# jhollowed/PyTEMDiags

Hardware: AMD Instinct MI355X
Metric: grid-points/sec through full TEM pipeline (ncol*nlev*nt) (higher is better)
Workload: dtype f64; 1 GPU; ne120 (777602 cols) x 72 lev x 30 snapshots per GPU, L=50, 1-degree zonal grid (M=180), ten GM16 Table-A1 outputs; ncol=777602, nlev=72, nt=30, sweeps=latitude-class, single sweep, mirror_paired_sweeps=True

## Files before the change

include/temx.h:

```cpp
#ifndef TEMX_H
#define TEMX_H

#include <stdint.h>

#ifdef __cplusplus
extern "C" {
#endif

typedef struct temx_plan temx_plan;

enum { TEMX_F64 = 0, TEMX_F32 = 1 };

enum {
  TEMX_OK = 0,
  TEMX_EINVAL = -1,
  TEMX_EHIP = -2,
  TEMX_ENOMEM = -3,
  TEMX_ERANK = -4,
  TEMX_ESTATE = -5,
  TEMX_EUNSUPPORTED = -6,
  TEMX_EINTERNAL = -7
};

enum {
  TEMX_DEFER_FINALIZE = 1,
  TEMX_NO_SYMMETRY = 2,
  TEMX_NO_CLASSES = 4,
  TEMX_NO_QR = 8,
  TEMX_LAT_TOL_F32 = 16
};

enum {
  TEMX_OPT_FORM = 1,
  TEMX_OPT_OS_MAP = 2,
  TEMX_OPT_OP_MAP = 3,
  TEMX_OPT_OS_SUBSAMPLE = 4,
  TEMX_OPT_TRACER_ONE_PASS = 5,
  TEMX_OPT_SINGLE_SWEEP_MIN_GROUPS = 6,
  TEMX_OPT_OS_CONTRACT = 7,
  TEMX_OPT_MISSING = 8,
  TEMX_OPT_MIN_COVERAGE = 9,
  TEMX_OPT_MISSING_WEIGHT = 10,
  TEMX_OPT_LAT_BINS = 12,
  TEMX_OPT_BIN_DEGREE = 13,
  TEMX_OPT_OS_SYNC = 11
};
enum {
  TEMX_FORM_AUTO = -1,
  TEMX_FORM_TWO_PASS = 0,
  TEMX_FORM_CLASS_SUMS = 1,
  TEMX_FORM_SINGLE_SWEEP = 2,
  TEMX_FORM_NO_SINGLE_SWEEP = 3,
  TEMX_FORM_MASKED = 4,
  TEMX_FORM_BINNED = 5
};

enum {
  TEMX_MAT_Y0 = 0,
  TEMX_MAT_Y0P = 1,
  TEMX_MAT_GRAM = 2,
  TEMX_MAT_GINV = 3,
  TEMX_MAT_Y0INV = 4,
  TEMX_MAT_GRAM2 = 5,
  TEMX_MAT_GX = 6,
  TEMX_MAT_GSUB = 7,
  TEMX_MAT_COVERAGE = 8
};

enum {
  TEMX_R_VTEM = 0, TEMX_R_OMEGATEM, TEMX_R_WTEM, TEMX_R_PSITEM, TEMX_R_EPFY, TEMX_R_EPFZ,
  TEMX_R_EPDIV, TEMX_R_UTENDEPFD, TEMX_R_UTENDVTEM, TEMX_R_UTENDWTEM, TEMX_NRESULTS
};

enum {
  TEMX_Z_UB = 0, TEMX_Z_VB, TEMX_Z_THETAB, TEMX_Z_WAPB, TEMX_Z_UPVPB, TEMX_Z_UPWAPPB,
  TEMX_Z_VPTPB, TEMX_Z_DUB_DP, TEMX_Z_DTHETAB_DP, TEMX_Z_UBCOSLAT, TEMX_Z_DUBCOSLAT_DLAT,
  TEMX_Z_PSI, TEMX_Z_PSICOSLAT, TEMX_Z_DPSICOSLAT_DLAT, TEMX_Z_DPSI_DP, TEMX_Z_INT_VBDP,
  TEMX_NZONAL
};

enum {
  TEMX_E_UP = 0, TEMX_E_VP, TEMX_E_THETAP, TEMX_E_WAPP, TEMX_E_UPVP, TEMX_E_UPWAPP, TEMX_E_VPTP,
  TEMX_NEDDY
};

int temx_version(void);
const char* temx_last_error(void);
int temx_device_count(void);

int temx_plan_create(temx_plan** out, int device, int64_t ncol, int L, int M,
                     const double* lat_deg_host, const double* lat_out_deg_host, int flags);

int temx_plan_finalize(temx_plan* plan, const double* G_host );

int temx_plan_refine(temx_plan* plan, const double* G2_host );

int temx_plan_set_weights(temx_plan* plan, const double* weights_host );

// ... 106 lines not shown
```

pytemdiags_amd/_lib.py:

```python
from __future__ import annotations

import ctypes as C
import os

_HERE = os.path.dirname(os.path.abspath(__file__))
LIB_PATH = os.environ.get("TEMX_LIB") or os.path.join(_HERE, "libtemx.so")

ABI_VERSION = 402
F64, F32 = 0, 1
DEFER_FINALIZE = 1
NO_SYMMETRY = 2
NO_CLASSES = 4
NO_QR = 8
LAT_TOL_F32 = 16
MAT_Y0, MAT_Y0P, MAT_GRAM, MAT_GINV, MAT_Y0INV, MAT_GRAM2, MAT_GX, MAT_GSUB = 0, 1, 2, 3, 4, 5, 6, 7
MAT_COVERAGE = 8
OPT_FORM, OPT_OS_MAP, OPT_OP_MAP, OPT_OS_SUBSAMPLE, OPT_TRACER_ONE_PASS, OPT_SINGLE_SWEEP_MIN_GROUPS, OPT_OS_CONTRACT = 1, 2, 3, 4, 5, 6, 7
OPT_MISSING, OPT_MIN_COVERAGE, OPT_MISSING_WEIGHT = 8, 9, 10
OPT_OS_SYNC = 11
OPT_LAT_BINS, OPT_BIN_DEGREE = 12, 13
LAT_BINS_ALLOWED = (128, 256, 512, 1024, 2048)
LAT_BINS_DEFAULT = 512
MISSING_MODES = {"raise": 0, "mask": 1}
FORM_AUTO, FORM_TWO_PASS, FORM_CLASS_SUMS, FORM_SINGLE_SWEEP, FORM_NO_SINGLE_SWEEP = -1, 0, 1, 2, 3
FORM_MASKED = 4
FORM_BINNED = 5
FORM_NAMES = {FORM_TWO_PASS: "two-pass", FORM_CLASS_SUMS: "class-sums", FORM_SINGLE_SWEEP: "single-sweep",
              FORM_MASKED: "masked", FORM_BINNED: "binned"}
FORMS = {"auto": FORM_AUTO, "two-pass": FORM_TWO_PASS, "class-sums": FORM_CLASS_SUMS,
         "single-sweep": FORM_SINGLE_SWEEP, "no-single-sweep": FORM_NO_SINGLE_SWEEP}

RESULT_NAMES = ("vtem", "omegatem", "wtem", "psitem", "epfy", "epfz", "epdiv",
                "utendepfd", "utendvtem", "utendwtem")
ZONAL_NAMES = ("ub", "vb", "thetab", "wapb", "upvpb", "upwappb", "vptpb", "dub_dp", "dthetab_dp",
               "ubcoslat", "dubcoslat_dlat", "psi", "psicoslat", "dpsicoslat_dlat", "dpsi_dp",
               "int_vbdp")
EDDY_NAMES = ("up", "vp", "thetap", "wapp", "upvp", "upwapp", "vptp")
TRACER_RESULT_NAMES = ("etfy", "etfz", "etdiv", "qtendetfd", "qtendvtem", "qtendwtem")
TRACER_ZONAL_NAMES = ("qb", "qpvpb", "qpwappb", "dqb_dp", "qbcoslat", "dqbcoslat_dlat")
TRACER_EDDY_NAMES = ("qp", "qpvp", "qpwapp")

ERRORS = {0: "TEMX_OK", -1: "TEMX_EINVAL", -2: "TEMX_EHIP", -3: "TEMX_ENOMEM", -4: "TEMX_ERANK",
          -5: "TEMX_ESTATE", -6: "TEMX_EUNSUPPORTED", -7: "TEMX_EINTERNAL"}

_vp, _i, _i64, _dp, _u64 = C.c_void_p, C.c_int, C.c_int64, C.POINTER(C.c_double), C.c_uint64
SIGNATURES = [
    ("temx_version", _i, []),
    ("temx_last_error", C.c_char_p, []),
    ("temx_device_count", _i, []),
    ("temx_plan_create", _i, [C.POINTER(_vp), _i, _i64, _i, _i, _dp, _dp, _i]),
    ("temx_plan_finalize", _i, [_vp, _dp]),
    ("temx_plan_refine", _i, [_vp, _dp]),
    ("temx_plan_set_weights", _i, [_vp, _dp]),
    ("temx_plan_destroy", None, [_vp]),
    ("temx_plan_is_paired", _i, [_vp]),
    ("temx_plan_sweep_mode", _i, [_vp]),
    ("temx_plan_one_pass", _i, [_vp]),
    ("temx_plan_single_sweep", _i, [_vp]),
    ("temx_get_matrix", _i, [_vp, _i, _vp, _vp]),
    ("temx_plan_configure", _i, [_vp, _i, _i]),
    ("temx_plan_option", _i, [_vp, _i]),
    ("temx_plan_set_os_matrices", _i, [_vp, _dp, _dp]),
    ("temx_project", _i, [_vp, _vp, _i, _i64, _vp, _vp]),
    ("temx_zonal_mean", _i, [_vp, _vp, _i, _i64, _vp, _i, _vp]),
    ("temx_zonal_mean_from_sums", _i, [_vp, _vp, _i64, _vp, _i, _vp]),
    ("temx_plan_set_tem", _i, [_vp, _i, _i64, _dp, C.c_double]),
    ("temx_tem_stage1", _i, [_vp, _vp, _vp, _vp, _vp, _i, _vp, _vp]),
    ("temx_tem_stage2", _i, [_vp, _vp, _vp, _vp, _vp, _i, _vp, _vp, _vp]),
    ("temx_tem_stage2_from_sums", _i, [_vp, _vp, _vp, _vp]),
    ("temx_tem_stage3", _i, [_vp, _vp, _vp, _vp, _vp]),
    ("temx_tem_run", _i, [_vp, _vp, _vp, _vp, _vp, _i, _vp, _vp, _vp]),
# ... 95 lines not shown
```

pytemdiags_amd/csrc/kernels_op2.hpp:

```cpp
#pragma once
#include "kernels_op.hpp"

namespace temx {

template <int NA, int NB>
struct OpwSlot {
  double sd[2][NA][64];
  double y[NB * 16];
};

template <int TBS, int NA>
__device__ __forceinline__ void opw_round(const OpwSlot<NA, 2 * TBS>* slots, int par, int t0, int nbw,
                                          uint32_t yoff, int lane, double (&acc)[NA][(TBS + 1) / 2]) {
  asm volatile("s_waitcnt lgkmcnt(0)\n\ts_barrier" ::: "memory");
#pragma unroll
  for (int j = 0; j < 4; ++j) {
    double b[NA];
#pragma unroll
    for (int f = 0; f < NA; ++f) b[f] = slots[j].sd[par][f][lane];
#pragma unroll
    for (int tl = 0; tl < (TBS + 1) / 2; ++tl)
      if (tl < nbw) {
        const double ya = slots[j].y[(t0 + tl) * 16 + yoff];
#pragma unroll
// ... 907 lines not shown
    }
  };

  if (b0 < b1) {
    load_ys(grp);
    rn = crow[(int64_t)b0 * 4 + wave];
    static_for<PD - 1>([&](auto kc) __attribute__((always_inline)) {
      constexpr int k = decltype(kc)::value;
      const int4 r0 = rn;
      rn = crow[(int64_t)(b0 + k + 1) * 4 + wave];
      issue(kc, r0);
    });
    constexpr int UNR = PD % 4 == 0 ? PD : PD % 2 == 0 ? 2 * PD : 4 * PD;
    for (int b = b0; b < b1; b += UNR)
      static_for<UNR>([&](auto kc) __attribute__((always_inline)) {
        constexpr int k = decltype(kc)::value;
        if (k == 0 || b + k < b1) step(kc, b + k);
      });
    asm volatile("s_waitcnt vmcnt(0)" ::: "memory");
  }
  if constexpr (SYNC != 0) {
    if (hpend) {
      if (left > 0) {
        const int first = (b1 - b0) & (NCH - 1);
        static_for<NCH>([&](auto cc) __attribute__((always_inline)) {
          if (((decltype(cc)::value - first) & (NCH - 1)) < left) pending_chunk(cc);
        });
      }
      handoff_wait(&hctr[0], handoff_look(&hctr[0]), 4u * hgen, 1);
      tile_role(ypend);
    }
    if (hfail != 0 && lane == 0) atomicOr(hstat, hfail);
  }
  if (left > 0) {
    const int first = (b1 - b0) & (NCH - 1);
    static_for<NCH>([&](auto cc) __attribute__((always_inline)) {
      if (((decltype(cc)::value - first) & (NCH - 1)) < left) pending_chunk(cc);
    });
  }
  if (dvalid) {
#pragma unroll
    for (int f = 0; f < NFX; ++f)
#pragma unroll
      for (int t = 0; t < NBX; ++t) {
        const int l = symx_harm<TBX>(t, g);
        if (l < (pp != nullptr ? KX : K4)) px[(((int64_t)split * NFX + f) * KX + l) * D + d] = ax[f][t];
      }
#pragma unroll
    for (int k = 0; k < NP; ++k)
#pragma unroll
      for (int t = 0; t < 2 * TBS; ++t) {
        const int l = sym_harm<TBS>(t, g);
        if (pp != nullptr && l < K) pp[(((int64_t)split * NP + k) * K + l) * D + d] = k < NPR ? apr[k < NPR ? k : 0][t] : apl[((k < NPR ? 0 : k - NPR) * 2 * TBS + t) * 64];
      }
  }
}

#ifndef TEMX_OS2_STAGGER
#define TEMX_OS2_STAGGER 0
#endif
#ifndef TEMX_OS2_ACC32
#define TEMX_OS2_ACC32 1
#endif
template <typename T, int TBS, int TBX, int NBR, int PD, int KIND = 0>
__global__ void __launch_bounds__(512, 1)
sweep_os2_kernel(FieldPtrs<4> fp, int64_t D, int K, int KX, const double* __restrict__ ycx,
                 const int4* __restrict__ crowN, const int4* __restrict__ crowS,
                 const int* __restrict__ gfirstN, const int* __restrict__ gfirstS, const int2* __restrict__ csplit,
                 const double* __restrict__ colscale, const double* __restrict__ rho, int K4,
                 double* __restrict__ px, double* __restrict__ pp, int nsplit, int ndt) {
  using KD = OsKind<KIND>;
  constexpr int NF = KD::NF, NFX = KD::NFX, NP = KD::NP;
  constexpr int NBX = 2 * TBX;
  constexpr int YE = NBX * 16;
  constexpr int MB = CLS_MB;
  constexpr int NCH = 2;
  constexpr int NV = NF + NP;
  constexpr int NPR = KD::NPR, NPL = NP - NPR;
  static_assert(NBR <= TBS && TBS <= TBX, "reference degree <= L <= 2L");
  static_assert(YE <= 512, "one Y element per thread");
  static_assert((PD - 1) * MB * NF + (MB - 1) * NF + 1 <= 63, "the ring is counted in vmcnt (6 bits)");
  extern __shared__ double lds[];
  int split, dq;
  if (!wg_work((ndt + 3) / 4, nsplit, split, dq)) return;
  const int tid = threadIdx.x;
  const int wave = uniform_wave(), lane = tid & 63;
  const int c = lane & 15, g = lane >> 4;
  const int side = wave >> 2;
  const int64_t colr = (int64_t)dq * 64 + lane < D ? (int64_t)dq * 64 + lane : D - 1;
  const uint32_t colb32 = (uint32_t)colr * (uint32_t)sizeof(T);
  const int tl = wave & 3, par = wave >> 2;
  const int dt = dq * 4 + tl;
  const int64_t d = (int64_t)dt * 16 + c;
  const bool dvalid = dt < ndt && d < D;
  const int64_t dcl = dvalid ? d : D - 1;
  const int4* __restrict__ crow = side ? crowS : crowN;
  const int* __restrict__ gfirst = side ? gfirstS : gfirstN;
  int grp = __builtin_amdgcn_readfirstlane(csplit[split].y);
  const int grp1 = __builtin_amdgcn_readfirstlane(csplit[split + 1].y);
  const int b0 = __builtin_amdgcn_readfirstlane(gfirst[grp]);
  const int b1 = __builtin_amdgcn_readfirstlane(gfirst[grp1]);
  const uint32_t aoff_p = (uint32_t)(g * 4 + (lane & 3));
  const uint32_t aoff_r = (uint32_t)((lane & 3) * 4 + g);
  double* ybase = lds;
  double* cn = lds + 2 * YE;
  double* cb = lds + 2 * YE + 16 + tl * (NF * 2 * NBR * 64) + lane;
// ... 660 lines not shown
```

pytemdiags_amd/csrc/temx.hip:

```cpp
#include "../../include/temx.h"
#include "../../include/temx_vert.h"
#include "../../include/temx_layout.h"
#include "../../include/temx_ingest.h"
#include "../../include/temx_clim.h"

#include <hip/hip_runtime.h>

#include <algorithm>
#include <cmath>
#include <cstdarg>
#include <cstdio>
#include <cstdlib>
#include <cstring>
#include <map>
#include <mutex>
#include <new>
#include <stdexcept>
#include <string>
#include <thread>
#include <atomic>
#include <vector>

#include "kernels.hpp"
#include "kernels_sym.hpp"
// ... 76 lines not shown
  bool finalized = false;
  bool weighted = false;
  int rank = 0;
  DevBuf x, Y0, yblk, yblk_w, Y0p, G, Ginv, norm, flag;
  DevBuf gblk, ypblk;
  bool qbasis = false;
  bool g_checker = false;
  bool ext_G = false;
  bool os_need_global = false;
  DevBuf T, Qp, GinvA, G2, xo, xc;
  int64_t cls_npad = 0;
  const double* yproj_ptr() const { return yblk_w.p ? yblk_w.d() : yblk.d(); }
  std::vector<double> lat_out_deg;
  bool tem = false;
  int nlev = 0;
  int64_t nt = 0, D = 0;
  double p0 = 101325.0;
  DevBuf p, pg, lg, coslat, fcor, colscale;
  DevBuf B4, B3, C4, zb;
  DevBuf Bq, Bq2, Ct, tz;
  Split sp_proj1;
  bool sym = false;
  int TBS = 0;
  int64_t npair = 0, npg = 0, npg_alloc = 0;
  DevBuf rows, ysym;
  Split sp_sproj4, sp_sproj1, sp_seddy;
  Split sp_proj4, sp_eddy;
  bool cls = false;
  int64_t cgroups = 0, cbatches = 0, ncls = 0;
  int64_t cls_max_side = 0;
  std::vector<int> gbatch0;
  DevBuf crow, ycls;
  std::map<int, DevBuf> csplits;
  Split sp_cproj4, sp_cproj1, sp_ceddy, sp_cflux;
  bool os_built = false, os_on = false;
  bool os_valid = false;
  DevBuf Axq, rho_t;
  int TBX = 0, KX = 0, KR = 0, NQ = 0;
  std::vector<double> h_xc, h_cnt;
  std::vector<int> h_crow;
  std::vector<int> sgbatch0;
  int64_t sgroups = 0, sbatches = 0;
  DevBuf ycx, ycx_s, crow_s, rho, rho0, gaunt , wq2, Gx, Gsinv, Ax , Axs ;
  std::vector<double> h_G_own;
  std::vector<double> h_Gx_own;
  std::vector<double> h_Gx, h_Gs;
  std::vector<double> h_T, h_Ginv, h_G, h_Yq;
  DevBuf oscblk, osAt, osAb, osAtq, osAbq, Bqp;
  OscMats osc{};
  bool osc_lds = false;
  int opt_os_contract = -1;
  bool os_barrier = false;
  int opt_os_sync = -1;
  int os_keep = 32;
  int64_t tD = 0, tnt = 0, tt0 = 0;
  int opt_form = -1, opt_os_map = -1, opt_op_map = -1, opt_tracer_one_pass = -1, opt_single_sweep_min_groups = -1;
  bool os_tile = false, op_tile = false;
  bool no_qr = false;
  DevBuf side_crow[2][2], side_gfirst[2][2];
  std::map<int, DevBuf> csplits_s;
  Split sp_os, sp_os_s;
  Split sp_copw;
  bool lcls = false, lone = false, xb_valid = false;
  DevBuf ycls_l, pbuf;
  int64_t ycls_lstride = 0;
  Split sp_lflux;
  bool onepass = false, op_valid = false;
  bool c4_valid = false;
  DevBuf csum, ccnt;
  DevBuf Pq;
  DevBuf csq, Pq2;
  bool tq_valid = false;
  DevBuf partial;
  DevBuf opB, opC;
  int opt_missing = 0, opt_min_cov = 500, opt_miss_w = 10;
  bool miss_built = false;
  bool miss_valid = false;
  int64_t miss_cov_D = -1;
  int NE = 0, NQM = 0;
  DevBuf eblk;
  DevBuf mtab;
  DevBuf mB, mC, mCcov, mcov, mZ;
  int opt_lat_bins = 0;
  int bin_J = 0, bin_KP = 0;
  int bin_built = 0;
  int bin_pass = 0;
  int64_t bin_nchunk = 0;
  std::vector<double> h_lat;
  DevBuf bin_a, bin_chunk, bin_c0, bin_rows, bin_s;
  DevBuf bin_T;
  DevBuf bin_cm, bin_z, bin_cy;
  bool timing = false;
  std::vector<TimedLaunch> timed[2];
};

static int upload(DevBuf& b, const void* src, size_t bytes) {
  int rc = b.ensure(bytes);
  if (rc) return rc;
  HIPCHK(hipMemcpy(b.p, src, bytes, hipMemcpyHostToDevice));
  return TEMX_OK;
}

__global__ void fill_zero_kernel(double2* __restrict__ p, int64_t n) {
  const double2 z = make_double2(0.0, 0.0);
  for (int64_t i = blockIdx.x * (int64_t)blockDim.x + threadIdx.x; i < n; i += (int64_t)gridDim.x * blockDim.x) p[i] = z;
}
// ... 940 lines not shown
}

static void set_tail(temx_plan* pl, int64_t t0, int64_t nts) {
  if (pl->tt0 != t0 || pl->tnt != nts) pl->c4_valid = pl->os_valid = pl->op_valid = pl->tq_valid = pl->xb_valid = false;
  pl->tt0 = t0;
  pl->tnt = nts;
  pl->tD = (int64_t)pl->nlev * nts;
}
static inline bool tail_is_whole(const temx_plan* pl) { return pl->tt0 == 0 && pl->tnt == pl->nt; }

static int tem_stage3_impl(temx_plan* pl, const double* B3, double* results, double* zonal, hipStream_t st);
static int tem_epilogue(temx_plan* pl, double* results, double* zonal, hipStream_t st);
static int bin_project_op(temx_plan* pl, const void* A, int dtype, int64_t D, double* B, hipStream_t st);
static int bin_zonal_mean(temx_plan* pl, const void* A, int dtype, int64_t D, double* out, int native, hipStream_t st);
static int miss_check(const temx_plan* pl);
static int miss_zonal_mean(temx_plan* pl, const void* A, int dtype, int64_t D, double* out, int native, hipStream_t st);
static int tracer_stage3_impl(temx_plan* pl, const double* Bq2, double* tres, double* tzon, hipStream_t st);

static SliceMap slice_map(const temx_plan* pl, int nsl, int64_t rows_total, int64_t row0) {
  SliceMap m;
  if (nsl <= 1) return m;
  m.D = pl->D;
  m.nt = (int)pl->nt;
  m.W = nsl;
  m.chunk = rows_total * pl->nlev * ((pl->nt + nsl - 1) / nsl);
  m.row0 = row0;
  return m;
}

template <int NBK>
static int launch_osc_t(temx_plan* pl, const OscFieldsIn& fin, int nf, int nout, double* Bf, double* At, double* ab,
                        const OscPairsIn& pin, int np, double* Bp, int64_t Dt, hipStream_t st) {
  const unsigned gx = (unsigned)((Dt + 15) / 16);
  hipLaunchKernelGGL((osc_fields_kernel<NBK>), dim3(gx, nf, 2), dim3(OSC_W * 64), (size_t)osc_fields_lds(NBK) * 8, st, fin, pl->osc, pl->K,
                     pl->KX, pl->KR, pl->NQ, Dt, nout, Bf, At, ab, pl->D, (int)pl->tnt, (int)pl->nt, (int)pl->tt0);
  HIPCHK(hipGetLastError());
  hipLaunchKernelGGL((osc_pairs_kernel<NBK>), dim3(gx, np), dim3(OSC_W * 64), (size_t)osc_pairs_lds(NBK) * 8, st, pin, pl->osc, pl->wq2.d(),
                     pl->K, pl->KX, pl->NQ, Dt, Bp);
  HIPCHK(hipGetLastError());
  return TEMX_OK;
}
static int launch_osc(temx_plan* pl, const OscFieldsIn& fin, int nf, int nout, double* Bf, double* At, double* ab,
                      const OscPairsIn& pin, int np, double* Bp, int64_t Dt, hipStream_t st) {
  if (pl->TB == 13 && pl->TBX == 13) return launch_osc_t<13>(pl, fin, nf, nout, Bf, At, ab, pin, np, Bp, Dt, st);
  if (pl->TB == 8 && pl->TBX == 8) return launch_osc_t<8>(pl, fin, nf, nout, Bf, At, ab, pin, np, Bp, Dt, st);
  if (pl->TB == 4 && pl->TBX == 4) return launch_osc_t<4>(pl, fin, nf, nout, Bf, At, ab, pin, np, Bp, Dt, st);
  return fail(TEMX_EUNSUPPORTED, "single-sweep contraction: no instantiation for L = %d", pl->L);
}

static int os_prepass(temx_plan* pl, const FieldPtrs<4>& fp, int dtype, double* As, hipStream_t st) {
  int rc;
  const int64_t D = pl->D, KD4 = (int64_t)4 * pl->KX * D;
  pl->op_valid = pl->c4_valid = pl->tq_valid = pl->os_valid = false;
  if ((rc = launch_sweep_os<0>(pl, fp, dtype, true, pl->rho0.d(), pl->partial.d(), pl->sp_os_s, st))) return rc;
  return launch_reduce_rows(pl, pl->partial.d(), pl->sp_os_s.nsplit, KD4, 4, pl->KX, pl->KR, D, As, st);
}

static int os_sweep(temx_plan* pl, const FieldPtrs<4>& fp, int dtype, const double* As, int nsl, double* proj, hipStream_t st) {
  int rc;
  const int64_t D = pl->D;
  const int64_t KD4 = (int64_t)4 * pl->KX * D, KD3 = (int64_t)3 * pl->K * D;
  pl->op_valid = pl->c4_valid = pl->tq_valid = pl->os_valid = false;
  hipLaunchKernelGGL(os_ref_solve_kernel, dim3((unsigned)((D + 15) / 16), 4), dim3(256), 0, st, As, pl->KR, pl->KR, D,
                     pl->Gsinv.d(), pl->rho.d());
  HIPCHK(hipGetLastError());
  TimedLaunch tl{};
  time_begin(pl, 0, st, tl);
  rc = launch_sweep_os<0>(pl, fp, dtype, false, pl->rho.d(), pl->partial.d(), pl->sp_os, st);
  time_end(pl, 0, st, tl);
  if (rc) return rc;
  const int64_t rows = (int64_t)4 * pl->KX + 3 * pl->K;
  if ((rc = launch_reduce(pl, pl->partial.d(), pl->sp_os.nsplit, KD4, proj, st, -1, nullptr, slice_map(pl, nsl, rows, 0)))) return rc;
  return launch_reduce(pl, pl->partial.d() + (int64_t)pl->sp_os.nsplit * KD4, pl->sp_os.nsplit, KD3, nsl > 1 ? proj : proj + KD4, st, -1,
                       nullptr, slice_map(pl, nsl, rows, (int64_t)4 * pl->KX));
}

static int os_tail(temx_plan* pl, const double* proj_s, int64_t t0, int64_t nts, double* results, double* zonal, hipStream_t st) {
  int rc;
  set_tail(pl, t0, nts);
  const int64_t Dt = pl->tD;
  const int64_t rows = (int64_t)4 * pl->KX + 3 * pl->K;
  if (proj_s != pl->Ax.d())
    HIPCHK(hipMemcpyAsync(pl->Ax.p, proj_s, (size_t)rows * Dt * 8, hipMemcpyDeviceToDevice, st));
  {
    TimedLaunch t2{};
    time_begin(pl, 1, st, t2);
    const size_t lds = os_contract_lds(pl->K, pl->KX, pl->NQ) * 8;
    static std::atomic<uint64_t> attr_set{0};
    if ((rc = lds_attr_once(attr_set, pl->device, reinterpret_cast<const void*>(os_contract_kernel<0>), 160 * 1024))) return rc;
    const double* Pp = pl->Ax.d() + (int64_t)4 * pl->KX * Dt;
    if (pl->osc_lds) {
      OsFields in;
      for (int f = 0; f < 4; ++f) {
        in.A[f] = pl->Ax.d() + (int64_t)f * pl->KX * Dt;
        in.rho[f] = pl->rho.d() + (int64_t)f * pl->KR * pl->D;
      }
      hipLaunchKernelGGL(os_contract_kernel<0>, dim3((unsigned)((Dt + OSC - 1) / OSC)), dim3(256), lds, st, in, Pp, pl->K, pl->KX,
                         pl->KR, pl->NQ, Dt, pl->T.d(), pl->Ginv.d(), pl->G.d(), pl->Gx.d(), pl->gaunt.d(), pl->wq2.d(),
                         pl->B4.d(), pl->B3.d(), pl->D, (int)nts, (int)pl->nt, (int)t0);
      HIPCHK(hipGetLastError());
    } else {
      using KD = OsKind<0>;
      const int64_t QD = (int64_t)pl->NQ * Dt;
      OscFieldsIn fin;
      OscPairsIn pin{};
      for (int f = 0; f < 4; ++f) {
        fin.A[f] = pl->Ax.d() + (int64_t)f * pl->KX * Dt;
// ... 905 lines not shown
                              void* stream) try {
  if (pl && miss_mode(pl)) return miss_refuse("temx_zonal_mean_from_sums");
  if (pl && bin_refused(pl)) return bin_refuse("temx_zonal_mean_from_sums");
  if (!pl || !B || !out) return fail(TEMX_EINVAL, "null argument");
  if (!pl->finalized) return fail(TEMX_ESTATE, "plan not finalised");
  HIPCHK(hipSetDevice(pl->device));
  int rc;
  if (!native) return launch_solve(pl, B, 1, D, nullptr, out, S_(stream));
  if ((rc = pl->opC.ensure((size_t)pl->K4 * D * 8))) return rc;
  if ((rc = launch_solve(pl, B, 1, D, pl->opC.d(), nullptr, S_(stream)))) return rc;
  return launch_recon(pl, D, pl->opC.d(), out, S_(stream));
} TEMX_CATCH

int temx_zonal_mean(temx_plan* pl, const void* A, int dtype, int64_t D, double* out, int native,
                    void* stream) try {
  if (!pl || !A || !out) return fail(TEMX_EINVAL, "null argument");
  if (!pl->finalized) return fail(TEMX_ESTATE, "plan not finalised");
  if (miss_mode(pl)) return miss_zonal_mean(pl, A, dtype, D, out, native, S_(stream));
  if (bin_mode(pl)) return bin_zonal_mean(pl, A, dtype, D, out, native, S_(stream));
  int rc = pl->opB.ensure((size_t)pl->K * std::max<int64_t>(D, 1) * 8);
  if (rc) return rc;
  if ((rc = temx_project(pl, A, dtype, D, pl->opB.d(), stream))) return rc;
  return temx_zonal_mean_from_sums(pl, pl->opB.d(), D, out, native, stream);
} TEMX_CATCH

struct FormChoice {
  bool two_pass;
  bool force_op;
  int os;
};
static FormChoice form_choice(const temx_plan* pl) {
  FormChoice c{false, false, -1};
  if (bin_mode(pl)) return FormChoice{true, false, 0};
  switch (pl->opt_form) {
    case TEMX_FORM_TWO_PASS: c.two_pass = true; c.os = 0; break;
    case TEMX_FORM_CLASS_SUMS: c.force_op = true; c.os = 0; break;
    case TEMX_FORM_SINGLE_SWEEP: c.force_op = true; c.os = 1; break;
    case TEMX_FORM_NO_SINGLE_SWEEP: c.os = 0; break;
    default: break;
  }
  if (const char* e = getenv("TEMX_TWO_PASS")) c.two_pass = e[0] == '1';
  if (const char* e = getenv("TEMX_ONE_PASS")) c.force_op = c.force_op || e[0] == '1';
  if (const char* e = getenv("TEMX_SINGLE_SWEEP")) c.os = e[0] == '0' ? 0 : (e[0] == '1' ? 1 : c.os);
  return c;
}
static bool tile_map(int opt, const char* env) {
  if (const char* e = getenv(env)) return !strcmp(e, "tile");
  return opt == 1;
}
static bool os_barrier_wanted(const temx_plan* pl) {
  if (const char* e = getenv("TEMX_OS_SYNC")) return !strcmp(e, "barrier");
  return pl->opt_os_sync == 1;
}
static bool tracer_one_pass_wanted(const temx_plan* pl) {
  if (const char* e = getenv("TEMX_TRACER_ONE_PASS")) return e[0] == '1';
  return pl->opt_tracer_one_pass == 1;
}

static int bin_check(const temx_plan* pl);
static int bin_set_tem(temx_plan* pl);

int temx_plan_configure(temx_plan* pl, int option, int value) try {
  if (!pl) return fail(TEMX_EINVAL, "null plan");
  switch (option) {
    case TEMX_OPT_FORM:
      if (value < -1 || value > TEMX_FORM_NO_SINGLE_SWEEP) return fail(TEMX_EINVAL, "TEMX_OPT_FORM: unknown form %d", value);
      pl->opt_form = value;
      break;
    case TEMX_OPT_OS_MAP: pl->opt_os_map = value; break;
    case TEMX_OPT_OP_MAP: pl->opt_op_map = value; break;
    case TEMX_OPT_TRACER_ONE_PASS: pl->opt_tracer_one_pass = value; break;
    case TEMX_OPT_OS_SUBSAMPLE:
      if (value < 4) return fail(TEMX_EINVAL, "TEMX_OPT_OS_SUBSAMPLE: at least 4 class-groups");
      if (pl->os_built && value != pl->os_keep) return fail(TEMX_ESTATE, "the single-sweep tables of this plan are built: set the subsample before temx_plan_set_tem");
      pl->os_keep = value;
      break;
    case TEMX_OPT_SINGLE_SWEEP_MIN_GROUPS: pl->opt_single_sweep_min_groups = value; break;
    case TEMX_OPT_OS_CONTRACT: pl->opt_os_contract = value; break;
    case TEMX_OPT_MISSING:
      if (value != 0 && value != 1) return fail(TEMX_EINVAL, "TEMX_OPT_MISSING: 0 (raise) or 1 (mask), got %d", value);
      if (value == 1) {
        if (bin_mode(pl)) return fail(TEMX_EUNSUPPORTED, "missing-value mode is not available while latitude bins are in effect (TEMX_OPT_LAT_BINS)");
        if (int rc = miss_check(pl)) return rc;
      }
      pl->opt_missing = value;
      pl->miss_valid = false;
      break;
    case TEMX_OPT_MIN_COVERAGE:
      if (value < 0 || value > 1000) return fail(TEMX_EINVAL, "TEMX_OPT_MIN_COVERAGE: per mille in 0..1000, got %d", value);
      pl->opt_min_cov = value;
      break;
    case TEMX_OPT_MISSING_WEIGHT:
      if (value < 4 || value > 14) return fail(TEMX_EINVAL, "TEMX_OPT_MISSING_WEIGHT: tau = 10^-value, value in 4..14, got %d", value);
      pl->opt_miss_w = value;
      break;
    case TEMX_OPT_OS_SYNC:
      if (value != 0 && value != 1) return fail(TEMX_EINVAL, "TEMX_OPT_OS_SYNC: 0 (flags) or 1 (barriers), got %d", value);
      pl->opt_os_sync = value;
      break;
    case TEMX_OPT_LAT_BINS: {
      const int B = value == -1 ? BIN_DEFAULT : value;
      if (B != 0) {
        if (!bin_count_ok(B)) return fail(TEMX_EINVAL, "TEMX_OPT_LAT_BINS: 0 (off), -1 (default, %d) or one of 128, 256, 512, 1024, 2048, got %d", BIN_DEFAULT, value);
        if (int rc = bin_check(pl)) return rc;
        if (bin_degree(pl->L, B) == 0)
          return fail(TEMX_EINVAL, "TEMX_OPT_LAT_BINS: (L, B) = (%d, %d): no Chebyshev degree up to %d keeps the basis rows to %.0e; use more bins",
                      pl->L, B, BIN_MAX_DEGREE, BIN_BOUND);
      }
      pl->opt_lat_bins = B;
      pl->bin_J = B ? bin_degree(pl->L, B) : 0;
      break;
    }
    case TEMX_OPT_BIN_DEGREE: return fail(TEMX_EINVAL, "TEMX_OPT_BIN_DEGREE is chosen by the library (read it with temx_plan_option)");
    default: return fail(TEMX_EINVAL, "unknown option %d", option);
  }
  pl->tem = false;
  return TEMX_OK;
} TEMX_CATCH

int temx_plan_option(const temx_plan* pl, int option) try {
  if (!pl) return -1;
  switch (option) {
    case TEMX_OPT_FORM:
      if (miss_mode(pl)) return TEMX_FORM_MASKED;
      if (bin_mode(pl)) return TEMX_FORM_BINNED;
      return pl->os_on ? TEMX_FORM_SINGLE_SWEEP : ((pl->cls && pl->onepass) || (pl->lcls && pl->lone) ? TEMX_FORM_CLASS_SUMS : TEMX_FORM_TWO_PASS);
    case TEMX_OPT_OS_MAP: return tile_map(pl->opt_os_map, "TEMX_OS_MAP") ? 1 : 0;
    case TEMX_OPT_OP_MAP: return tile_map(pl->opt_op_map, "TEMX_OP_MAP") ? 1 : 0;
    case TEMX_OPT_TRACER_ONE_PASS: return tracer_one_pass_wanted(pl) ? 1 : 0;
    case TEMX_OPT_OS_SUBSAMPLE: return pl->os_keep;
    case TEMX_OPT_SINGLE_SWEEP_MIN_GROUPS: return pl->opt_single_sweep_min_groups;
    case TEMX_OPT_OS_CONTRACT: return pl->osc_lds ? 1 : 0;
    case TEMX_OPT_MISSING: return pl->opt_missing;
    case TEMX_OPT_MIN_COVERAGE: return pl->opt_min_cov;
    case TEMX_OPT_MISSING_WEIGHT: return pl->opt_miss_w;
    case TEMX_OPT_OS_SYNC: return os_barrier_wanted(pl) ? 1 : 0;
    case TEMX_OPT_LAT_BINS: return pl->opt_lat_bins;
    case TEMX_OPT_BIN_DEGREE: return pl->bin_J;
    default: return -1;
  }
} TEMX_CATCH

int temx_plan_set_tem(temx_plan* pl, int nlev, int64_t nt, const double* p_pa_host, double p0) try {
  if (!pl || !p_pa_host) return fail(TEMX_EINVAL, "null argument");
  if (nlev < 2 || nt < 1) return fail(TEMX_EINVAL, "need nlev >= 2 and nt >= 1");
  if ((int64_t)nlev * nt >= ((int64_t)1 << 28)) return fail(TEMX_EINVAL, "nlev*nt must be < 2^28");
  if (pl->M < 2) return fail(TEMX_EINVAL, "need at least 2 zonal-mean latitudes");
  HIPCHK(hipSetDevice(pl->device));
  std::vector<double> p(p_pa_host, p_pa_host + nlev);
  for (int j = 1; j < nlev; ++j)
    if (!(p[j] > p[j - 1])) return fail(TEMX_EINVAL, "pressure must be strictly ascending (front end flips)");
  pl->tem = false;
  pl->onepass = pl->lone = pl->op_valid = pl->xb_valid = pl->tq_valid = false;
  pl->os_on = pl->os_valid = false;
  pl->os_tile = tile_map(pl->opt_os_map, "TEMX_OS_MAP");
  {
    const char* e = getenv("TEMX_OS_CONTRACT");
    pl->osc_lds = e ? !strcmp(e, "lds") : pl->opt_os_contract == 1;
  }
  pl->op_tile = tile_map(pl->opt_op_map, "TEMX_OP_MAP");
  pl->os_barrier = os_barrier_wanted(pl);
  pl->nlev = nlev;
  pl->nt = nt;
  pl->D = (int64_t)nlev * nt;
  pl->tD = pl->D;
  pl->tnt = nt;
  pl->tt0 = 0;
  pl->p0 = p0;
  const int M = pl->M;
  const int64_t D = pl->D;
  int rc;
  const TemTables tt = tem_tables(p, nt, p0, pl->lat_out_deg);
  if ((rc = upload(pl->p, p))) return rc;
  if ((rc = upload(pl->pg, tt.pg))) return rc;
  if ((rc = upload(pl->lg, tt.lg))) return rc;
  if ((rc = upload(pl->coslat, tt.coslat))) return rc;
  if ((rc = upload(pl->fcor, tt.fcor))) return rc;
  if ((rc = upload(pl->colscale, tt.colscale))) return rc;

  const int ndt_ = (int)((D + 15) / 16);
  const int pdpw = proj_dpw(4, ndt_);
  pl->sp_proj4 = choose_split(D, pl->nchunk, proj_wps(4, pdpw) * pl->num_cu, pdpw);
  const int edpw = pick_dpw(ndt_, 4);
  pl->sp_eddy = choose_split(D, pl->nchunk / (8 / edpw), pl->num_cu, edpw);
  const size_t need =
      (size_t)std::max(pl->sp_proj4.nsplit * 4, pl->sp_eddy.nsplit * (8 / edpw) * 3) * pl->K * D * 8;
  if ((rc = pl->partial.ensure(need))) return rc;
  if ((rc = pl->B4.ensure((size_t)4 * pl->K * D * 8))) return rc;
  if ((rc = pl->B3.ensure((size_t)3 * pl->K * D * 8))) return rc;
  if ((rc = pl->C4.ensure((size_t)4 * pl->K4 * D * 8))) return rc;
  if ((rc = pl->zb.ensure((size_t)8 * M * D * 8))) return rc;
  pl->sp_proj1 = choose_split(D, pl->nchunk, 2 * pl->num_cu);
  if (unfused_stage2(pl)) {
    const size_t need3 = (size_t)pl->sp_proj1.nsplit * 3 * 64 * D * 8;
    if ((rc = pl->partial.ensure(std::max(need3, pl->partial.bytes)))) return rc;
  }
  pl->lone = false;
  pl->xb_valid = false;
  pl->op_valid = false;
  if (pl->lcls) {
    const size_t need_cs = (size_t)pl->cgroups * ndt_ * 14 * 64 * 8, need_pb = (size_t)pl->cgroups * ndt_ * 3 * 128 * 8;
    size_t fr = 0, tot = 0;
    if (ndt_ >= 4 && !form_choice(pl).two_pass && hipMemGetInfo(&fr, &tot) == hipSuccess &&
        (pl->csum.bytes >= need_cs || need_cs + need_pb < fr / 2) && alloc_write_stream(pl->csum, need_cs) == TEMX_OK &&
        pl->pbuf.ensure(need_pb) == TEMX_OK) {
      HIPCHK(hipMemset(pl->csum.p, 0, pl->csum.bytes));
      HIPCHK(hipMemset(pl->pbuf.p, 0, pl->pbuf.bytes));
      const int64_t cunits = std::max<int64_t>(1, pl->cbatches / 4);
      pl->sp_cproj4 = choose_split(D, cunits, TEMX_CLS_OP_WPS * pl->num_cu, 4, 8);
      pl->sp_cflux = choose_split(D, std::max<int64_t>(1, pl->cgroups / (8 / edpw)), pl->num_cu, edpw, TEMX_CLS_MINCHUNK);
      pl->sp_lflux = choose_split(D, std::max<int64_t>(1, pl->cgroups / 8), pl->num_cu, 1, TEMX_CLS_MINCHUNK);
      const size_t need4 = (size_t)pl->sp_cflux.nsplit * 4 * 64 * D * 8;
      if ((rc = pl->partial.ensure(std::max(need4, pl->partial.bytes)))) return rc;
      if ((rc = pl->Bs.ensure((size_t)4 * 64 * D * 8))) return rc;
// ... 1339 lines not shown
```

pytemdiags_amd/engine.py:

```python
from __future__ import annotations

import ctypes as C

import numpy as np
import torch

from . import _lib
from ._lib import check

_DT = {torch.float64: _lib.F64, torch.float32: _lib.F32}


def _ptr(t):
    return C.c_void_p(t.data_ptr())


def _dbl(a):
    a = np.ascontiguousarray(a, dtype=np.float64)
    return a, a.ctypes.data_as(C.POINTER(C.c_double))


def lat_bins_value(lat_bins):
    if lat_bins is None or lat_bins is False:
        return 0
# ... 3 lines not shown
        return int(lat_bins)
    raise ValueError("lat_bins must be True, 0 or one of %s, got %r" % (_lib.LAT_BINS_ALLOWED, lat_bins))


class Plan:

    def __init__(self, lat_deg, lat_out_deg, L, device=0, defer_finalize=False, symmetry=True, classes=True, qr=True,
                 form=None, fp32_fields=False, lat_bins=None):
        self._h = C.c_void_p()
        self.lib = _lib.load()
        if isinstance(device, torch.device):
            device = device.index or 0
        self.device_index = int(device)
        self.device = torch.device("cuda", self.device_index)
        lat, plat = _dbl(lat_deg)
        lat_out, plat_out = _dbl(lat_out_deg)
        self.N, self.M, self.L, self.K = int(lat.size), int(lat_out.size), int(L), int(L) + 1
        self.lat_out = lat_out
        self.nlev = self.nt = self.D = None
        self.form_requested = "auto"
        check(self.lib.temx_plan_create(C.byref(self._h), self.device_index, self.N, self.L, self.M,
                                        plat, plat_out, (_lib.DEFER_FINALIZE if defer_finalize else 0)
                                        | (0 if symmetry else _lib.NO_SYMMETRY)
                                        | (0 if classes else _lib.NO_CLASSES)
                                        | (0 if qr else _lib.NO_QR)
                                        | (_lib.LAT_TOL_F32 if fp32_fields else 0)))
        if form is not None:
            self.configure(form=form)
        if lat_bins is not None:
            self.configure(lat_bins=lat_bins)

    @property
    def paired(self):
        return bool(self.lib.temx_plan_is_paired(self._h))

    @property
    def sweep_mode(self):
        return int(self.lib.temx_plan_sweep_mode(self._h))

    @property
    def one_pass(self):
        return bool(self.lib.temx_plan_one_pass(self._h))

    @property
    def single_sweep(self):
        return bool(self.lib.temx_plan_single_sweep(self._h))

    @property
    def tracer_one_pass(self):
        return self.one_pass and self.option(_lib.OPT_TRACER_ONE_PASS) == 1

    def configure(self, form=None, os_map=None, op_map=None, os_subsample=None, tracer_one_pass=None,
                  single_sweep_min_groups=None, os_contract=None, missing=None, min_coverage=None,
                  missing_weight=None, os_sync=None, lat_bins=None):
        def put(opt, val):
            check(self.lib.temx_plan_configure(self._h, opt, int(val)))
        if missing is not None:
            if missing not in _lib.MISSING_MODES:
                raise ValueError("missing must be 'raise' or 'mask', got %r" % (missing,))
            put(_lib.OPT_MISSING, _lib.MISSING_MODES[missing])
        if min_coverage is not None:
            mc = float(min_coverage)
            if not 0.0 <= mc <= 1.0:
                raise ValueError("min_coverage must lie in [0, 1], got %r" % (min_coverage,))
            put(_lib.OPT_MIN_COVERAGE, int(round(mc * 1000)))
        if missing_weight is not None:
            e = -np.log10(float(missing_weight))
            if not (float(missing_weight) > 0 and abs(e - round(e)) < 1e-9 and 4 <= round(e) <= 14):
                raise ValueError("missing_weight must be 10^-n with n in 4..14, got %r" % (missing_weight,))
            put(_lib.OPT_MISSING_WEIGHT, int(round(e)))
        if form is not None:
            put(_lib.OPT_FORM, _lib.FORMS[form] if isinstance(form, str) else form)
            self.form_requested = form
        for opt, val in ((_lib.OPT_OS_MAP, os_map), (_lib.OPT_OP_MAP, op_map)):
            if val is not None:
                put(opt, {"row": 0, "tile": 1}[val] if isinstance(val, str) else val)
        if os_subsample is not None:
            put(_lib.OPT_OS_SUBSAMPLE, os_subsample)
        if tracer_one_pass is not None:
            put(_lib.OPT_TRACER_ONE_PASS, 1 if tracer_one_pass else 0)
        if single_sweep_min_groups is not None:
            put(_lib.OPT_SINGLE_SWEEP_MIN_GROUPS, single_sweep_min_groups)
        if os_contract is not None:
            put(_lib.OPT_OS_CONTRACT, {"mfma": 0, "lds": 1}[os_contract] if isinstance(os_contract, str) else os_contract)
        if lat_bins is not None:
            put(_lib.OPT_LAT_BINS, lat_bins_value(lat_bins))
        if os_sync is not None:
            put(_lib.OPT_OS_SYNC, {"flags": 0, "barrier": 1}[os_sync] if isinstance(os_sync, str) else os_sync)
        self.nlev = self.nt = self.D = None

    def option(self, opt):
        return int(self.lib.temx_plan_option(self._h, int(opt)))

    @property
    def lat_bins(self):
        return self.option(_lib.OPT_LAT_BINS)

    @property
    def bin_degree(self):
        return self.option(_lib.OPT_BIN_DEGREE)

    @property
    def sweep_form(self):
        return _lib.FORM_NAMES.get(self.option(_lib.OPT_FORM), "two-pass")

    @property
    def missing(self):
        return "mask" if self.option(_lib.OPT_MISSING) == 1 else "raise"

    def coverage(self):
        D = getattr(self, "_cov_D", None) or self.D or 1
        out = torch.empty((self.M, D), dtype=torch.float64, device=self.device)
        check(self.lib.temx_get_matrix(self._h, _lib.MAT_COVERAGE, _ptr(out), self._stream()))
        return out

    def close(self):
        if getattr(self, "_h", None) is not None and self._h.value:
            self.lib.temx_plan_destroy(self._h)
            self._h = C.c_void_p()

    def __del__(self):
        try:
            self.close()
        except Exception:
            pass

    def _stream(self):
        return C.c_void_p(torch.cuda.current_stream(self.device).cuda_stream)

    def _field(self, A, D=None):
        if not isinstance(A, torch.Tensor):
            raise TypeError("device tensors expected")
        if A.device != self.device:
            raise ValueError("tensor on %s, plan on %s" % (A.device, self.device))
        if A.dtype not in _DT:
            raise TypeError("dtype must be float64 or float32, got %s" % A.dtype)
        if A.shape[0] != self.N:
            raise ValueError("leading dimension must be ncol = %d" % self.N)
        A = A.contiguous()
        if D is not None and A.numel() != self.N * D:
            raise ValueError("field has %d elements, expected %d x %d" % (A.numel(), self.N, D))
# ... 447 lines not shown
```

Measured before the change: 188.6 billion grid-points/s.

## Add dedicated lean pre-pass kernel for single-sweep OS prepass in f64

Adds a specialized prepass_osr_kernel that computes north/south class means of the four fields and contracts them against the Y basis with MFMA, replacing the generic sweep kernel used as the pre-pass for f64 row-mapped plans. It uses a deeper software-pipelined ring of row loads counted in vmcnt and a lighter per-group exchange through LDS. The aim is to cut register pressure and work in the pre-pass. It is on by default and can be disabled with an option or environment variable. Risk: correctness depends on matching the class-flag handling of the old path, and occupancy may change.

```diff
diff --git a/include/temx.h b/include/temx.h
--- a/include/temx.h
+++ b/include/temx.h
@@ -43,7 +43,8 @@
   TEMX_OPT_MISSING_WEIGHT = 10,
   TEMX_OPT_LAT_BINS = 12,
   TEMX_OPT_BIN_DEGREE = 13,
-  TEMX_OPT_OS_SYNC = 11
+  TEMX_OPT_OS_SYNC = 11,
+  TEMX_OPT_OS_LEAN = 14
 };
 enum {
   TEMX_FORM_AUTO = -1,
diff --git a/pytemdiags_amd/_lib.py b/pytemdiags_amd/_lib.py
--- a/pytemdiags_amd/_lib.py
+++ b/pytemdiags_amd/_lib.py
@@ -17,6 +17,7 @@
 MAT_COVERAGE = 8
 OPT_FORM, OPT_OS_MAP, OPT_OP_MAP, OPT_OS_SUBSAMPLE, OPT_TRACER_ONE_PASS, OPT_SINGLE_SWEEP_MIN_GROUPS, OPT_OS_CONTRACT = 1, 2, 3, 4, 5, 6, 7
 OPT_MISSING, OPT_MIN_COVERAGE, OPT_MISSING_WEIGHT = 8, 9, 10
+OPT_OS_LEAN = 14
 OPT_OS_SYNC = 11
 OPT_LAT_BINS, OPT_BIN_DEGREE = 12, 13
 LAT_BINS_ALLOWED = (128, 256, 512, 1024, 2048)
diff --git a/pytemdiags_amd/csrc/kernels_op2.hpp b/pytemdiags_amd/csrc/kernels_op2.hpp
--- a/pytemdiags_amd/csrc/kernels_op2.hpp
+++ b/pytemdiags_amd/csrc/kernels_op2.hpp
@@ -983,6 +983,179 @@
       for (int t = 0; t < 2 * TBS; ++t) {
         const int l = sym_harm<TBS>(t, g);
         if (pp != nullptr && l < K) pp[(((int64_t)split * NP + k) * K + l) * D + d] = k < NPR ? apr[k < NPR ? k : 0][t] : apl[((k < NPR ? 0 : k - NPR) * 2 * TBS + t) * 64];
+      }
+  }
+}
+
+template <typename T, int NBR, int PD>
+__global__ void __launch_bounds__(256, 2)
+prepass_osr_kernel(FieldPtrs<4> fp, int64_t D, int KX, int TBX, const double* __restrict__ ycx,
+                   const int4* __restrict__ crow, const int2* __restrict__ csplit,
+                   const double* __restrict__ colscale, int K4, double* __restrict__ px, int nsplit, int ndt) {
+  constexpr int NF = 4, TF = 2;
+  constexpr int MB = CLS_MB;
+  constexpr int NY = 2 * NBR;
+  static_assert((PD - 1) * MB * NF + (MB - 1) * NF + NY <= 63, "the ring is counted in vmcnt (6 bits)");
+  __shared__ double ex[2 * NF * 256];
+  __shared__ double cn[8];
+  int split, dq;
+  if (!wg_work((ndt + 3) / 4, nsplit, split, dq)) return;
+  const int tid = threadIdx.x;
+  const int wave = uniform_wave(), lane = tid & 63;
+  const int c = lane & 15, g = lane >> 4;
+  const int64_t colr = (int64_t)dq * 64 + lane < D ? (int64_t)dq * 64 + lane : D - 1;
+  const uint32_t colb32 = (uint32_t)colr * (uint32_t)sizeof(T);
+  const int dt = dq * 4 + wave;
+  const int64_t d = (int64_t)dt * 16 + c;
+  const bool dvalid = dt < ndt && d < D;
+  const int b0 = __builtin_amdgcn_readfirstlane(csplit[split].x);
+  const int b1 = __builtin_amdgcn_readfirstlane(csplit[split + 1].x);
+  int grp = __builtin_amdgcn_readfirstlane(csplit[split].y);
+  const uint32_t aoff_p = (uint32_t)(g * 4 + (lane & 3));
+  double* exw = ex + wave * 64 + lane;
+  const double* exr = ex + g * 64 + wave * 16 + c;
+  const double sth = colscale != nullptr ? colscale[colr] : 1.0;
+  uint64_t fbase[NF];
+#pragma unroll
+  for (int f = 0; f < NF; ++f) fbase[f] = reinterpret_cast<uint64_t>(fp.p[f]);
+  { double sth_ready = sth; asm volatile("" : "+v"(sth_ready)); }
+
+  double ax[NF][NY];
+#pragma unroll
+  for (int f = 0; f < NF; ++f)
+#pragma unroll
+    for (int t = 0; t < NY; ++t) ax[f][t] = 0.0;
+  double s[NF], x0[NF], sN[NF], x0N[NF];
+  int cnt = 0, cntN = 0;
+#pragma unroll
+  for (int f = 0; f < NF; ++f) s[f] = x0[f] = sN[f] = x0N[f] = 0.0;
+  bool north_open = false, prev_south = false;
+  const uint32_t rowbytes = (uint32_t)D * (uint32_t)sizeof(T);
+  const uint32_t ybytes = (uint32_t)(2 * TBX * 16 * 8);
+
+  T xb[PD][MB][NF];
+  int er[PD][MB];
+  double ys[NY];
+  uint32_t yoff32[NY];
+#pragma unroll
+  for (int t = 0; t < NY; ++t) yoff32[t] = (uint32_t)((t < NBR ? t : TBX + (t - NBR)) * 16 + (int)aoff_p) * 8u;
+  auto load_ys = [&](int gi) __attribute__((always_inline)) {
+#pragma unroll
+    for (int t = 0; t < NY; ++t) RowLoad<double>::ld(ys[t], yoff32[t], reinterpret_cast<uint64_t>(ycx) + (uint64_t)gi * ybytes);
+  };
+  auto issue = [&](auto pc, const int4 rv) __attribute__((always_inline)) {
+    constexpr int P = decltype(pc)::value;
+    er[P][0] = rv.x; er[P][1] = rv.y; er[P][2] = rv.z; er[P][3] = rv.w;
+#pragma unroll
+    for (int j = 0; j < MB; ++j) {
+      const uint64_t off = (uint64_t)(uint32_t)(er[P][j] & CLS_ROWMASK) * rowbytes;
+#pragma unroll
+      for (int f = 0; f < NF; ++f) RowLoad<T>::ld(xb[P][j][f], colb32, fbase[f] + off);
+    }
+  };
+  auto park_north = [&]() __attribute__((always_inline)) {
+#pragma unroll
+    for (int f = 0; f < NF; ++f) { sN[f] = s[f]; x0N[f] = x0[f]; s[f] = 0.0; }
+    cntN = cnt;
+    cnt = 0;
+  };
+  int4 rn;
+  auto step = [&](auto posc, int b) __attribute__((always_inline)) {
+    constexpr int P = decltype(posc)::value % PD;
+    {
+      const int4 r1 = rn;
+      rn = crow[(int64_t)(b + PD) * 4 + wave];
+      issue(std::integral_constant<int, (P + PD - 1) % PD>{}, r1);
+    }
+    static_for<MB>([&](auto jc) __attribute__((always_inline)) {
+      constexpr int j = decltype(jc)::value;
+      constexpr int NW = (PD - 1) * MB * NF + (MB - 1 - j) * NF;
+      row_wait<NW>(xb[P][j][0], xb[P][j][1], xb[P][j][2], xb[P][j][3]);
+    });
+#pragma unroll
+    for (int t = 0; t < NY; ++t) row_touch(ys[t]);
+    const int fl = er[P][0] >> 27;
+    const bool south = (fl & (CLS_SOUTH << 1)) != 0;
+    if ((fl & (CLS_FIRST << 1)) || (south && !prev_south)) {
+      if (south && north_open) park_north();
+      north_open = !south;
+#pragma unroll
+      for (int f = 0; f < NF; ++f) x0[f] = (double)xb[P][0][f];
+    }
+    prev_south = south;
+#pragma unroll
+    for (int j = 0; j < MB; ++j)
+      if (er[P][j] >= 0) {
+#pragma unroll
+        for (int f = 0; f < NF; ++f) s[f] += (double)xb[P][j][f] - x0[f];
+        cnt += 1;
+      }
+    if (fl & (CLS_LAST << 1)) {
+      prev_south = false;
+      if (north_open) park_north();
+      north_open = false;
+      const double nNd = (double)cntN, nSd = (double)cnt;
+      const double rnN = nNd > 0.0 ? temx_rcp_count(nNd) : 0.0, rnS = nSd > 0.0 ? temx_rcp_count(nSd) : 0.0;
+      double val[2 * NF];
+#pragma unroll
+      for (int f = 0; f < NF; ++f) {
+        const double sc = f == TF ? sth : 1.0;
+        val[f] = (sN[f] * rnN + x0N[f]) * sc;
+        val[NF + f] = (s[f] * rnS + x0[f]) * sc;
+      }
+      asm volatile("s_waitcnt lgkmcnt(0)\n\ts_barrier" ::: "memory");
+#pragma unroll
+      for (int v = 0; v < 2 * NF; ++v) exw[v * 256] = val[v];
+      if (lane == 0) {
+        cn[wave] = nNd;
+        cn[4 + wave] = nSd;
+      }
+      asm volatile("s_waitcnt lgkmcnt(0)\n\ts_barrier" ::: "memory");
+      static_assert(NY == 4, "row_wait has forms for 3 and 4 values");
+      row_wait<MB * NF>(ys[0], ys[1], ys[2], ys[3]);
+      const double nN = cn[g], nS = cn[4 + g];
+      double dS[NF][2];
+#pragma unroll
+      for (int f = 0; f < NF; ++f) {
+        const double SNf = nN * exr[f * 256], SSf = nS * exr[(NF + f) * 256];
+        dS[f][0] = SNf + SSf;
+        dS[f][1] = SNf - SSf;
+      }
+#pragma unroll
+      for (int t = 0; t < NY; ++t)
+#pragma unroll
+        for (int f = 0; f < NF; ++f) ax[f][t] = TEMX_MFMA4(ys[t], dS[f][t < NBR ? 0 : 1], ax[f][t]);
+      ++grp;
+      load_ys(grp);
+#pragma unroll
+      for (int f = 0; f < NF; ++f) s[f] = sN[f] = 0.0;
+      cnt = cntN = 0;
+    }
+  };
+
+  if (b0 < b1) {
+    load_ys(grp);
+    rn = crow[(int64_t)b0 * 4 + wave];
+    static_for<PD - 1>([&](auto kc) __attribute__((always_inline)) {
+      constexpr int k = decltype(kc)::value;
+      const int4 r0 = rn;
+      rn = crow[(int64_t)(b0 + k + 1) * 4 + wave];
+      issue(kc, r0);
+    });
+    for (int b = b0; b < b1; b += PD)
+      static_for<PD>([&](auto kc) __attribute__((always_inline)) {
+        constexpr int k = decltype(kc)::value;
+        if (k == 0 || b + k < b1) step(kc, b + k);
+      });
+    asm volatile("s_waitcnt vmcnt(0)" ::: "memory");
+  }
+  if (dvalid) {
+#pragma unroll
+    for (int f = 0; f < NF; ++f)
+#pragma unroll
+      for (int t = 0; t < NY; ++t) {
+        const int l = t < NBR ? 2 * (4 * t + g) : 2 * (4 * (t - NBR) + g) + 1;
+        if (l < K4) px[(((int64_t)split * NF + f) * KX + l) * D + d] = ax[f][t];
       }
   }
 }
diff --git a/pytemdiags_amd/csrc/temx.hip b/pytemdiags_amd/csrc/temx.hip
--- a/pytemdiags_amd/csrc/temx.hip
+++ b/pytemdiags_amd/csrc/temx.hip
@@ -152,6 +152,8 @@
   int opt_os_contract = -1;
   bool os_barrier = false;
   int opt_os_sync = -1;
+  bool os_lean = true;
+  int opt_os_lean = -1;
   int os_keep = 32;
   int64_t tD = 0, tnt = 0, tt0 = 0;
   int opt_form = -1, opt_os_map = -1, opt_op_map = -1, opt_tracer_one_pass = -1, opt_single_sweep_min_groups = -1;
@@ -1198,7 +1200,16 @@
   int rc;
   const int64_t D = pl->D, KD4 = (int64_t)4 * pl->KX * D;
   pl->op_valid = pl->c4_valid = pl->tq_valid = pl->os_valid = false;
-  if ((rc = launch_sweep_os<0>(pl, fp, dtype, true, pl->rho0.d(), pl->partial.d(), pl->sp_os_s, st))) return rc;
+  if (dtype == TEMX_F64 && pl->os_lean && !pl->os_tile) {
+    const Split& sp = pl->sp_os_s;
+    const int2* cuts = nullptr;
+    if ((rc = os_cuts_dev(pl, true, sp.nsplit, &cuts))) return rc;
+    hipLaunchKernelGGL((prepass_osr_kernel<double, 2, 2>), dim3(sp.grid), dim3(256), 0, st, fp, D, pl->KX, pl->TBX, pl->ycx_s.d(),
+                       static_cast<const int4*>(pl->crow_s.p), cuts, pl->colscale.d(), pl->KR, pl->partial.d(), sp.nsplit, sp.ndt);
+    HIPCHK(hipGetLastError());
+  } else if ((rc = launch_sweep_os<0>(pl, fp, dtype, true, pl->rho0.d(), pl->partial.d(), pl->sp_os_s, st))) {
+    return rc;
+  }
   return launch_reduce_rows(pl, pl->partial.d(), pl->sp_os_s.nsplit, KD4, 4, pl->KX, pl->KR, D, As, st);
 }
 
@@ -2210,6 +2221,10 @@
   if (const char* e = getenv("TEMX_OS_SYNC")) return !strcmp(e, "barrier");
   return pl->opt_os_sync == 1;
 }
+static bool os_lean_wanted(const temx_plan* pl) {
+  if (const char* e = getenv("TEMX_OS_LEAN")) return e[0] != '1';
+  return pl->opt_os_lean != 1;
+}
 static bool tracer_one_pass_wanted(const temx_plan* pl) {
   if (const char* e = getenv("TEMX_TRACER_ONE_PASS")) return e[0] == '1';
   return pl->opt_tracer_one_pass == 1;
@@ -2256,6 +2271,10 @@
       if (value != 0 && value != 1) return fail(TEMX_EINVAL, "TEMX_OPT_OS_SYNC: 0 (flags) or 1 (barriers), got %d", value);
       pl->opt_os_sync = value;
       break;
+    case TEMX_OPT_OS_LEAN:
+      if (value != 0 && value != 1) return fail(TEMX_EINVAL, "TEMX_OPT_OS_LEAN: 0 (pre-pass kernel of its own) or 1 (the sweep kernel as the pre-pass), got %d", value);
+      pl->opt_os_lean = value;
+      break;
     case TEMX_OPT_LAT_BINS: {
       const int B = value == -1 ? BIN_DEFAULT : value;
       if (B != 0) {
@@ -2293,6 +2312,7 @@
     case TEMX_OPT_MIN_COVERAGE: return pl->opt_min_cov;
     case TEMX_OPT_MISSING_WEIGHT: return pl->opt_miss_w;
     case TEMX_OPT_OS_SYNC: return os_barrier_wanted(pl) ? 1 : 0;
+    case TEMX_OPT_OS_LEAN: return os_lean_wanted(pl) ? 0 : 1;
     case TEMX_OPT_LAT_BINS: return pl->opt_lat_bins;
     case TEMX_OPT_BIN_DEGREE: return pl->bin_J;
     default: return -1;
@@ -2318,6 +2338,7 @@
   }
   pl->op_tile = tile_map(pl->opt_op_map, "TEMX_OP_MAP");
   pl->os_barrier = os_barrier_wanted(pl);
+  pl->os_lean = os_lean_wanted(pl);
   pl->nlev = nlev;
   pl->nt = nt;
   pl->D = (int64_t)nlev * nt;
diff --git a/pytemdiags_amd/engine.py b/pytemdiags_amd/engine.py
--- a/pytemdiags_amd/engine.py
+++ b/pytemdiags_amd/engine.py
@@ -79,7 +79,7 @@
 
     def configure(self, form=None, os_map=None, op_map=None, os_subsample=None, tracer_one_pass=None,
                   single_sweep_min_groups=None, os_contract=None, missing=None, min_coverage=None,
-                  missing_weight=None, os_sync=None, lat_bins=None):
+                  missing_weight=None, os_sync=None, lat_bins=None, os_lean=None):
         def put(opt, val):
             check(self.lib.temx_plan_configure(self._h, opt, int(val)))
         if missing is not None:
@@ -114,6 +114,8 @@
             put(_lib.OPT_LAT_BINS, lat_bins_value(lat_bins))
         if os_sync is not None:
             put(_lib.OPT_OS_SYNC, {"flags": 0, "barrier": 1}[os_sync] if isinstance(os_sync, str) else os_sync)
+        if os_lean is not None:
+            put(_lib.OPT_OS_LEAN, int(os_lean))
         self.nlev = self.nt = self.D = None
 
     def option(self, opt):
```

New measurement: 189.4 billion grid-points/s, median of 2. No clear change (+0.4%).
